# openclimatefix/predict_pv_yield

Hardware: AMD Instinct MI355X
Metric: PV-site samples/sec (train step), conv3d 12->6 frames (higher is better)
Workload: dtype bf16; 1 GPU; conv3d train step (fwd + NMAE + bwd + Adam): sat [B,11,18,64,64] N(0,1), 4x Conv3d(3x3x3, 32ch) + fc 128/128/64, 128.6 M params; per_gpu_batch=32, global_batch=32, t_frames=18, parallelism=single

## Files before the change

include/pv_yield_hip.h:

```cpp
#ifndef PV_YIELD_HIP_H
#define PV_YIELD_HIP_H

#include <stddef.h>
#include <stdint.h>

#ifdef __cplusplus
extern "C" {
#endif

#define PV_ABI_VERSION 1

enum {
  PV_OK = 0,
  PV_EINVAL = -1,
  PV_ESIZE = -2,
  PV_ELAUNCH = -3
};

enum { PV_BORDER_CONSTANT = 0, PV_BORDER_REPLICATE = 1 };

enum {
  PV_U8_ROUND_DIV4 = 0,
  PV_U8_TRUNC_SCALE = 1
};
// ... 481 lines not shown
int pv_layernorm_bwd_workspace_bytes(int64_t rows, int32_t d, size_t* bytes);
int pv_layernorm_bwd_f32(const float* x, const float* w, const float* dy, const float* mean, const float* rstd, float* dx,
                         float* dw, float* db, int64_t rows, int32_t d, void* ws, size_t ws_bytes, int32_t accumulate,
                         const float* dx_add, void* stream);
int pv_layernorm_bwd_params_from_proj_workspace_bytes(int64_t rows, int32_t d, size_t* bytes);
int pv_layernorm_bwd_params_from_proj_bf16(const uint16_t* dkv16, const float* w_kv, const float* x, const float* mean,
                                           const float* rstd, float* dw, float* db, int64_t rows, int32_t d, int32_t kdim,
                                           void* ws, size_t ws_bytes, int32_t accumulate, void* stream);
int pv_context_fwd_bf16(const float* x, const float* x2, int32_t d1, int64_t period, const float* ln_w, const float* ln_b,
                        const float* w_kv, uint16_t* kv16, float* mean, float* rstd, int64_t rows, int32_t d, int32_t kdim,
                        float eps, void* stream);
int pv_context_bwd_workspace_bytes(int64_t rows, int32_t d, size_t* bytes);
int pv_context_bwd_bf16(const uint16_t* dkv16, const float* w_kv, const float* x, const float* x2, int32_t d1, int64_t period,
                        const float* mean, const float* rstd, const float* ln_w, const float* ln_b, float* dw_kv, float* dln_w,
                        float* dln_b, int64_t rows, int32_t d, int32_t kdim, void* ws, size_t ws_bytes, int32_t accumulate_kv,
                        int32_t accumulate_ln, void* stream);
int pv_softmax_fwd_f32(const float* x, float* y, int64_t rows, int32_t len, float scale, void* stream);
int pv_softmax_bwd_f32(const float* p, const float* dp, float* dx, int64_t rows, int32_t len, float scale, void* stream);
int pv_geglu_fwd_f32(const float* x, float* y, int64_t rows, int32_t h, void* stream);
int pv_geglu_bwd_f32(const float* x, const float* dy, float* dx, int64_t rows, int32_t h, void* stream);
int pv_mean_axis1_fwd_f32(const float* x, float* y, int32_t b, int32_t n, int32_t d, void* stream);
int pv_mean_axis1_bwd_f32(const float* dy, float* dx, int32_t b, int32_t n, int32_t d, void* stream);

int pv_gru_seq_fwd_f32(const float* gi, const float* h0, const float* w_hh, const float* b_hh, float* out, float* saved,
                       int32_t batch, int32_t t_len, int32_t hidden, void* stream);
int pv_gru_seq_bwd_f32(const float* dout, const float* dh_last, const float* h0, const float* out, const float* saved,
                       const float* w_hh, float* dgi, float* dh0, float* dw_hh, float* db_hh, int32_t batch, int32_t t_len,
                       int32_t hidden, void* ws, size_t ws_bytes, void* stream);

int pv_forecast_losses_f32(const float* y_hat, const float* y, int64_t y_row_stride,
                           int64_t y_col_stride, int32_t m, int32_t n, float grad_scale,
                           float* out4, float* grad, float* per_horizon, void* stream);

int pv_adam_step_f32(float* param, const float* grad, float* exp_avg, float* exp_avg_sq,
                     uint16_t* bf16_shadow, size_t n, double lr, double beta1, double beta2,
                     double eps, int32_t step, float grad_scale, void* stream);

int pv_ssim_mean_u8(const uint8_t* im1, int64_t stride1, const uint8_t* im2, int64_t stride2, int64_t n_pairs, int32_t h,
                    int32_t w, double data_range, double* out, void* stream);
int pv_ssim_mean_f32(const float* im1, int64_t stride1, const float* im2, int64_t stride2, int64_t n_pairs, int32_t h,
                     int32_t w, double data_range, double* out, void* stream);

int pv_stage_timing_begin(void);
int pv_stage_timing_end(const char** names, float* ms, int32_t* counts, int32_t capacity, int32_t* n_out);

int pv_calibrate_copy_f32(const float* src, float* dst, size_t n, void* stream);
int pv_calibrate_mfma_bf16(float* sink, int32_t workgroups, int32_t iters, void* stream);

int pv_clock_watch(unsigned long long* samples, int32_t n_samples, int32_t sleep_units, void* stream);

#ifdef __cplusplus
}
#endif
#endif
```

predict_pv_yield_amd/_lib.py:

```python
import ctypes
import os
import subprocess

_PKG = os.path.dirname(os.path.abspath(__file__))
LIB_PATH = os.environ.get("PV_YIELD_LIB") or os.path.join(_PKG, "lib", "libpvyield_hip.so")
CSRC_DIR = os.path.join(_PKG, "csrc")

PV_BORDER_CONSTANT = 0
PV_BORDER_REPLICATE = 1
PV_U8_ROUND_DIV4 = 0
PV_U8_TRUNC_SCALE = 1
PV_OPTFLOW_FARNEBACK_GAUSSIAN = 256

c_i32, c_i64, c_f32, c_f64 = ctypes.c_int32, ctypes.c_int64, ctypes.c_float, ctypes.c_double
c_vp, c_sz, c_int, c_u8 = ctypes.c_void_p, ctypes.c_size_t, ctypes.c_int, ctypes.c_uint8


class FarnebackParams(ctypes.Structure):
    _fields_ = [("pyr_scale", c_f64), ("levels", c_i32), ("winsize", c_i32), ("iterations", c_i32),
                ("poly_n", c_i32), ("poly_sigma", c_f64), ("flags", c_i32)]


class Conv3dDims(ctypes.Structure):
    _fields_ = [("batch", c_i32), ("c_in", c_i32), ("c_out", c_i32), ("t_in", c_i32), ("h_in", c_i32),
                ("w_in", c_i32), ("pad_t", c_i32), ("pad_h", c_i32), ("pad_w", c_i32)]

    def out_shape(self):
        return (self.t_in + 2 * self.pad_t - 2, self.h_in + 2 * self.pad_h - 2, self.w_in + 2 * self.pad_w - 2)


class AdamTensor(ctypes.Structure):
    _fields_ = [("param", c_vp), ("grad", c_vp), ("exp_avg", c_vp), ("exp_avg_sq", c_vp), ("bf16_shadow", c_vp),
                ("n", ctypes.c_uint64)]


class PackJob(ctypes.Structure):
    _fields_ = [("w", c_vp), ("wp", c_vp), ("c_out", c_i32), ("c_in", c_i32), ("transpose_flip", c_i32)]


class GemmDesc(ctypes.Structure):
# ... 199 lines not shown
    "pv_attention_fwd_f32": [c_vp, c_vp, c_vp, c_vp, c_vp, ctypes.POINTER(AttentionDesc), c_vp],
    "pv_attention_bwd_f32": [c_vp, c_vp, c_vp, c_vp, c_vp, c_vp, c_vp, c_vp, c_vp, c_vp, ctypes.POINTER(AttentionDesc), c_vp],
    "pv_attention_fwd_bf16": [c_vp, c_vp, c_vp, c_vp, c_vp, ctypes.POINTER(AttentionDesc), c_vp, c_vp],
    "pv_attention_fwd_bf16kv": [c_vp, c_vp, c_vp, c_vp, c_vp, ctypes.POINTER(AttentionDesc), c_vp, c_vp],
    "pv_attention_fwd_workspace_floats": [ctypes.POINTER(AttentionDesc)],
    "pv_attention_bwd_bf16": [c_vp, c_vp, c_vp, c_vp, c_vp, c_vp, c_vp, c_vp, c_vp, c_vp, ctypes.POINTER(AttentionDesc), c_i32, c_vp],
    "pv_attention_bwd_bf16kv": [c_vp, c_vp, c_vp, c_vp, c_vp, c_vp, c_vp, c_vp, c_vp, c_vp, ctypes.POINTER(AttentionDesc), c_i32, c_vp],
    "pv_attention_bwd_bf16kv16": [c_vp, c_vp, c_vp, c_vp, c_vp, c_vp, c_vp, c_vp, c_vp, c_vp, ctypes.POINTER(AttentionDesc), c_vp],
    "pv_attention_bwd_workspace_floats": [ctypes.POINTER(AttentionDesc)],
    "pv_layernorm_fwd_f32": [c_vp, c_vp, c_vp, c_vp, c_vp, c_vp, c_i64, c_i32, c_f32, c_vp],
    "pv_layernorm_bwd_workspace_bytes": [c_i64, c_i32, ctypes.POINTER(c_sz)],
    "pv_layernorm_bwd_f32": [c_vp, c_vp, c_vp, c_vp, c_vp, c_vp, c_vp, c_vp, c_i64, c_i32, c_vp, c_sz, c_i32, c_vp, c_vp],
    "pv_context_fwd_bf16": [c_vp, c_vp, c_i32, c_i64, c_vp, c_vp, c_vp, c_vp, c_vp, c_vp, c_i64, c_i32, c_i32, ctypes.c_float, c_vp],
    "pv_context_bwd_workspace_bytes": [c_i64, c_i32, ctypes.POINTER(c_sz)],
    "pv_context_bwd_bf16": [c_vp, c_vp, c_vp, c_vp, c_i32, c_i64, c_vp, c_vp, c_vp, c_vp, c_vp, c_vp, c_vp, c_i64, c_i32, c_i32,
                            c_vp, c_sz, c_i32, c_i32, c_vp],
    "pv_layernorm_bwd_params_from_proj_workspace_bytes": [c_i64, c_i32, ctypes.POINTER(c_sz)],
    "pv_layernorm_bwd_params_from_proj_bf16": [c_vp, c_vp, c_vp, c_vp, c_vp, c_vp, c_vp, c_i64, c_i32, c_i32, c_vp, c_sz, c_i32, c_vp],
    "pv_softmax_fwd_f32": [c_vp, c_vp, c_i64, c_i32, c_f32, c_vp],
    "pv_softmax_bwd_f32": [c_vp, c_vp, c_vp, c_i64, c_i32, c_f32, c_vp],
    "pv_geglu_fwd_f32": [c_vp, c_vp, c_i64, c_i32, c_vp],
    "pv_geglu_bwd_f32": [c_vp, c_vp, c_vp, c_i64, c_i32, c_vp],
    "pv_mean_axis1_fwd_f32": [c_vp, c_vp, c_i32, c_i32, c_i32, c_vp],
    "pv_mean_axis1_bwd_f32": [c_vp, c_vp, c_i32, c_i32, c_i32, c_vp],
    "pv_gru_seq_fwd_f32": [c_vp, c_vp, c_vp, c_vp, c_vp, c_vp, c_i32, c_i32, c_i32, c_vp],
    "pv_gru_seq_bwd_f32": [c_vp, c_vp, c_vp, c_vp, c_vp, c_vp, c_vp, c_vp, c_vp, c_vp, c_i32, c_i32, c_i32, c_vp, c_sz, c_vp],
    "pv_embedding_fwd_f32": [c_vp, c_vp, c_vp, c_i32, c_i32, c_i32, c_vp],
    "pv_embedding_bwd_f32": [c_vp, c_vp, c_vp, c_i32, c_i32, c_i32, c_vp],
    "pv_cast_f32_to_bf16": [c_vp, c_vp, c_sz, c_vp],
    "pv_scale_bias_relu_f32": [c_vp, c_vp, c_vp, c_i32, c_i32, c_f32, c_i32, c_vp],
    "pv_relu_gate_f32": [c_vp, c_vp, c_vp, c_sz, c_vp],
    "pv_relu_gate_max_f32": [c_vp, c_vp, c_vp, c_sz, c_vp, c_vp],
    "pv_forecast_losses_f32": [c_vp, c_vp, c_i64, c_i64, c_i32, c_i32, c_f32, c_vp, c_vp, c_vp, c_vp],
    "pv_adam_step_f32": [c_vp, c_vp, c_vp, c_vp, c_vp, c_sz, c_f64, c_f64, c_f64, c_f64, c_i32, c_f32, c_vp],
}
_RESTYPES = {"pv_last_error": ctypes.c_char_p, "pv_conv3d_packed_weight_elems": c_sz, "pv_conv3d_split2_weight_elems": c_sz,
             "pv_linear_fwd_f32_skinny_workspace_bytes": c_sz,
             "pv_attention_bwd_workspace_floats": c_sz, "pv_colsum_workspace_floats": c_sz,
             "pv_attention_fwd_workspace_floats": c_sz}


def build_library(verbose: bool = False) -> str:
    args = ["make", "-C", CSRC_DIR, "-j8"]
    if not verbose:
        args.append("-s")
    subprocess.check_call(args)
    return LIB_PATH


_lib = None


def get_lib():
    global _lib
    if _lib is None:
        if not os.path.exists(LIB_PATH):
            raise RuntimeError(
                f"{LIB_PATH} not found: the HIP extension is not built. Run `python -c 'import __graft_entry__ as g; "
                f"g.build()'` (or `make -C {CSRC_DIR}`). predict_pv_yield_amd has no CPU fallback.")
        import torch
        lib = ctypes.CDLL(LIB_PATH)
        for name, argtypes in SIGNATURES.items():
            fn = getattr(lib, name)
            fn.argtypes = argtypes
            fn.restype = _RESTYPES.get(name, c_int)
        if lib.pv_abi_version() != 1:
# ... 37 lines not shown
```

predict_pv_yield_amd/csrc/dense_f32.hip:

```cpp
#include "adam.h"

namespace pv {

__global__ __launch_bounds__(256) void swap01_segments_kernel(const u32x4* __restrict__ src, u32x4* __restrict__ dst, long long n0,
                                                               long long n1, long long seg16) {
  const size_t total = (size_t)n0 * n1 * seg16, stride = (size_t)gridDim.x * blockDim.x;
  for (size_t i = (size_t)blockIdx.x * blockDim.x + threadIdx.x; i < total; i += stride) {
    const size_t seg = i / seg16, c = i - seg * seg16;
    const size_t i1 = seg / n0, i0 = seg - i1 * n0;
    dst[i] = src[(i0 * n1 + i1) * seg16 + c];
  }
}

constexpr int M_TILE = 8;
constexpr long long SMALL_K = 4096, SMALL_MN = 1 << 16;

__global__ __launch_bounds__(256) void linear_fwd_partial_f32(const float* __restrict__ x,
                                                               const float* __restrict__ w,
                                                               float* __restrict__ partial, int m, int n,
                                                               long long k, long long k_chunk) {
  const int col = blockIdx.x;
  const int ks = blockIdx.y;
  const int m0 = blockIdx.z * M_TILE;
  const long long k0 = (long long)ks * k_chunk;
// ... 235 lines not shown
}

__device__ __forceinline__ void linear_bwd_db_body(const float* __restrict__ dy, const float* __restrict__ ymask,
                                                   float* __restrict__ db, int m, int n, int bx) {
  int col = bx * blockDim.x + threadIdx.x;
  if (col >= n) return;
  float s = 0.f;
  for (int r = 0; r < m; ++r) {
    size_t off = (size_t)r * n + col;
    float v = dy[off];
    if (ymask && !(ymask[off] > 0.f)) v = 0.f;
    s += v;
  }
  db[col] = s;
}

__global__ __launch_bounds__(256) void linear_bwd_small_f32(const float* __restrict__ x, const float* __restrict__ w,
                                                             const float* __restrict__ dy, const float* __restrict__ ymask,
                                                             float* __restrict__ dx, float* __restrict__ dw,
                                                             float* __restrict__ db, int m, int n, long long k, int kb,
                                                             int n_dx, int n_dw) {
  extern __shared__ float g[];
  int blk = blockIdx.x;
  if (blk < n_dx) {
    linear_bwd_dx_body(g, w, dy, ymask, dx, m, n, k, blk % kb, blk / kb);
  } else if (blk < n_dx + n_dw) {
    blk -= n_dx;
    linear_bwd_dw_body(g, x, dy, ymask, dw, m, n, k, blk % kb, blk / kb);
  } else {
    linear_bwd_db_body(dy, ymask, db, m, n, blk - n_dx - n_dw);
  }
}

__global__ __launch_bounds__(256) void linear_fwd_small_f32(const float* __restrict__ x, const float* __restrict__ w,
                                                             const float* __restrict__ bias, float* __restrict__ y, int m,
                                                             int n, int k, int relu) {
  const int i = blockIdx.x * blockDim.x + threadIdx.x;
  if (i >= m * n) return;
  const int r = i / n, col = i - r * n;
  const float* xr = x + (size_t)r * k;
  const float* wr = w + (size_t)col * k;
  float s0 = 0.f, s1 = 0.f, s2 = 0.f, s3 = 0.f;
  int kk = 0;
  if ((((uintptr_t)xr | (uintptr_t)wr) & 15) == 0) {
    for (; kk + 64 <= k; kk += 64) {
      f32x4 xv[16], wv[16];
#pragma unroll
      for (int j = 0; j < 16; ++j) xv[j] = *reinterpret_cast<const f32x4*>(xr + kk + 4 * j), wv[j] = *reinterpret_cast<const f32x4*>(wr + kk + 4 * j);
#pragma unroll
      for (int j = 0; j < 16; ++j) {
        s0 = fmaf(xv[j][0], wv[j][0], s0);
        s1 = fmaf(xv[j][1], wv[j][1], s1);
        s2 = fmaf(xv[j][2], wv[j][2], s2);
        s3 = fmaf(xv[j][3], wv[j][3], s3);
      }
    }
    for (; kk + 32 <= k; kk += 32) {
      f32x4 xv[8], wv[8];
#pragma unroll
      for (int j = 0; j < 8; ++j) xv[j] = *reinterpret_cast<const f32x4*>(xr + kk + 4 * j), wv[j] = *reinterpret_cast<const f32x4*>(wr + kk + 4 * j);
#pragma unroll
      for (int j = 0; j < 8; ++j) {
        s0 = fmaf(xv[j][0], wv[j][0], s0);
        s1 = fmaf(xv[j][1], wv[j][1], s1);
        s2 = fmaf(xv[j][2], wv[j][2], s2);
        s3 = fmaf(xv[j][3], wv[j][3], s3);
      }
    }
  }
  for (; kk + 4 <= k; kk += 4) {
    s0 = fmaf(xr[kk], wr[kk], s0);
    s1 = fmaf(xr[kk + 1], wr[kk + 1], s1);
    s2 = fmaf(xr[kk + 2], wr[kk + 2], s2);
    s3 = fmaf(xr[kk + 3], wr[kk + 3], s3);
  }
  for (; kk < k; ++kk) s0 = fmaf(xr[kk], wr[kk], s0);
  float s = (s0 + s1) + (s2 + s3);
  if (bias) s += bias[col];
  if (relu) s = s > 0.f ? s : 0.f;
  y[i] = s;
}

struct LossWeights { float w[64]; };

__global__ __launch_bounds__(256) void forecast_losses_f32(const float* __restrict__ y_hat, const float* __restrict__ y,
                                                            long long y_row_stride, long long y_col_stride, int m,
                                                            int n, float grad_scale, LossWeights lw,
                                                            float* __restrict__ out4, float* __restrict__ grad,
                                                            float* __restrict__ per_horizon) {
  float s_se = 0.f, s_ae = 0.f, s_wse = 0.f, s_wae = 0.f;
  const int total = m * n;
  const float inv = 1.0f / (float)total;
  for (int i = threadIdx.x; i < total; i += blockDim.x) {
    int r = i / n, c = i - r * n;
    float d = y_hat[i] - y[(long long)r * y_row_stride + (long long)c * y_col_stride];
    float a = fabsf(d);
    s_se += d * d;
    s_ae += a;
    s_wse += lw.w[c] * (d * d);
    s_wae += lw.w[c] * a;
    if (grad) grad[i] = (d > 0.f ? 1.f : (d < 0.f ? -1.f : 0.f)) * inv * grad_scale;
  }
  __shared__ float red[4][4];
  float v[4] = {s_se, s_ae, s_wse, s_wae};
#pragma unroll
  for (int q = 0; q < 4; ++q) {
    float t = v[q];
#pragma unroll
    for (int off = 32; off > 0; off >>= 1) t += __shfl_down(t, off, 64);
    if ((threadIdx.x & 63) == 0) red[threadIdx.x >> 6][q] = t;
  }
  __syncthreads();
  if (threadIdx.x < 4) {
    int q = threadIdx.x;
    out4[q] = (((red[0][q] + red[1][q]) + red[2][q]) + red[3][q]) * inv;
  }
  if (per_horizon && (int)threadIdx.x < n) {
    const int c = threadIdx.x;
    float se = 0.f, ae = 0.f;
    for (int r = 0; r < m; ++r) {
      float d = y_hat[r * n + c] - y[(long long)r * y_row_stride + (long long)c * y_col_stride];
      se += d * d;
      ae += fabsf(d);
    }
    per_horizon[c] = se / (float)m;
    per_horizon[n + c] = ae / (float)m;
  }
}

template <typename GT>
__global__ __launch_bounds__(256) void adam_step_f32(float* __restrict__ p, const GT* __restrict__ g,
                                                      float* __restrict__ m, float* __restrict__ v,
                                                      uint16_t* __restrict__ shadow, size_t n, AdamScalars ad,
                                                      float grad_scale) {
  size_t stride = (size_t)gridDim.x * blockDim.x * 4;
  for (size_t i = ((size_t)blockIdx.x * blockDim.x + threadIdx.x) * 4; i < n; i += stride) {
    if (i + 4 <= n) {
      f32x4 pv4 = *reinterpret_cast<const f32x4*>(p + i);
      f32x4 gv4;
      if constexpr (sizeof(GT) == 4) {
        gv4 = *reinterpret_cast<const f32x4*>(g + i);
      } else {
        const u32x2 raw = *reinterpret_cast<const u32x2*>(g + i);
        gv4[0] = __builtin_bit_cast(float, raw[0] << 16); gv4[1] = __builtin_bit_cast(float, raw[0] & 0xffff0000u);
        gv4[2] = __builtin_bit_cast(float, raw[1] << 16); gv4[3] = __builtin_bit_cast(float, raw[1] & 0xffff0000u);
      }
      f32x4 mv4 = *reinterpret_cast<const f32x4*>(m + i);
      f32x4 vv4 = *reinterpret_cast<const f32x4*>(v + i);
      uint16_t sh[4];
#pragma unroll
      for (int j = 0; j < 4; ++j) {
        float mm = mv4[j], vv = vv4[j], pp = pv4[j];
        adam_update(pp, mm, vv, gv4[j] * grad_scale, ad);
        mv4[j] = mm; vv4[j] = vv; pv4[j] = pp;
        sh[j] = f32_to_bf16_bits(pp);
      }
      *reinterpret_cast<f32x4*>(p + i) = pv4;
      *reinterpret_cast<f32x4*>(m + i) = mv4;
      *reinterpret_cast<f32x4*>(v + i) = vv4;
      if (shadow) {
// ... 98 lines not shown
    float mm = mv[j], v2 = vv[j], pp = pv[j];
    adam_update(pp, mm, v2, gv[j] * grad_scale, ad);
    mv[j] = mm, vv[j] = v2, pv[j] = pp;
    sh[j] = f32_to_bf16_bits(pp);
  }
  if (cnt == 4) {
    *reinterpret_cast<f32x4*>(T.param + i0) = *reinterpret_cast<const f32x4*>(pv);
    *reinterpret_cast<f32x4*>(T.exp_avg + i0) = *reinterpret_cast<const f32x4*>(mv);
    *reinterpret_cast<f32x4*>(T.exp_avg_sq + i0) = *reinterpret_cast<const f32x4*>(vv);
    if (T.bf16_shadow) {
      const u32x2 o = {(uint32_t)sh[0] | ((uint32_t)sh[1] << 16), (uint32_t)sh[2] | ((uint32_t)sh[3] << 16)};
      *reinterpret_cast<u32x2*>(T.bf16_shadow + i0) = o;
    }
  } else {
    for (int j = 0; j < cnt; ++j) {
      T.param[i0 + j] = pv[j], T.exp_avg[i0 + j] = mv[j], T.exp_avg_sq[i0 + j] = vv[j];
      if (T.bf16_shadow) T.bf16_shadow[i0 + j] = sh[j];
    }
  }
}

constexpr long long GEMM_K = 1 << 16;

static long long fwd_k_chunk(long long k, int* k_splits) {
  long long chunk = k >= GEMM_K ? 2048 : 8192;
  long long splits = (k + chunk - 1) / chunk;
  if (splits > 512) { splits = 512; chunk = (k + splits - 1) / splits; }
  if (splits < 1) splits = 1;
  splits = (k + chunk - 1) / chunk;
  *k_splits = (int)splits;
  return chunk;
}

}

using namespace pv;

extern "C" {

int pv_linear_workspace_bytes(int32_t m, int32_t n, int64_t k, size_t* bytes) {
  PV_REQUIRE(bytes && m > 0 && n > 0 && k > 0, PV_EINVAL, "pv_linear_workspace_bytes: bad arguments");
  int ks;
  fwd_k_chunk(k, &ks);
  *bytes = (size_t)ks * m * n * sizeof(float);
  return PV_OK;
}

int pv_linear_fwd_f32(const float* x, const float* w, const float* bias, float* y, int32_t m, int32_t n, int64_t k,
                      int relu, void* workspace, size_t workspace_bytes, void* stream) {
  PV_REQUIRE(x && w && y && workspace, PV_EINVAL, "pv_linear_fwd_f32: null pointer");
  PV_REQUIRE(m > 0 && n > 0 && k > 0, PV_EINVAL, "pv_linear_fwd_f32: bad sizes");
  int ks;
  long long chunk = fwd_k_chunk(k, &ks);
  PV_REQUIRE(workspace_bytes >= (size_t)ks * m * n * sizeof(float), PV_ESIZE, "pv_linear_fwd_f32: workspace too small");
  PV_REQUIRE(n <= 65535 && ks <= 65535, PV_ESIZE, "pv_linear_fwd_f32: n too large");
  hipStream_t st = as_stream(stream);
  if (k <= SMALL_K && (long long)m * n <= SMALL_MN) {
    hipLaunchKernelGGL(linear_fwd_small_f32, dim3((unsigned)((m * n + 255) / 256)), dim3(256), 0, st, x, w, bias, y, m, n, (int)k,
                       relu ? 1 : 0);
    return check_launch("pv_linear_fwd_f32");
  }
  if (k >= GEMM_K && k < (1ll << 31)) {
    pv_gemm_desc d = {m, n, (int32_t)k, k, 1, 1, k, n, 1, 1, 0, 0, 0, 0, 0, 0, ks, (int64_t)m * n};
    const int rc = pv_gemm_f32(x, w, nullptr, (float*)workspace, &d, 0, stream);
    if (rc != PV_OK) return rc;
  } else if (k % 4 == 0 && chunk % 4 == 0 && ((uintptr_t)x % 16) == 0 && ((uintptr_t)w % 16) == 0) {
// ... 41 lines not shown
  if (db) {
    hipLaunchKernelGGL(linear_bwd_db_f32, dim3((unsigned)((n + 255) / 256)), dim3(256), 0, st, dy, y_relu_mask, db, m, n);
  }
  return check_launch("pv_linear_bwd_f32");
}

int pv_relu_gate_f32(const float* dy, const float* y, float* out, size_t n, void* stream) {
  PV_REQUIRE(dy && y && out, PV_EINVAL, "pv_relu_gate_f32: null pointer");
  PV_REQUIRE(n % 4 == 0 && ((uintptr_t)dy % 16) == 0 && ((uintptr_t)y % 16) == 0 && ((uintptr_t)out % 16) == 0, PV_EINVAL,
             "pv_relu_gate_f32: 16-byte aligned buffers of a multiple of 4 elements");
  if (n == 0) return PV_OK;
  hipLaunchKernelGGL(relu_gate_f32_kernel, dim3(stream_grid(n / 4, 256)), dim3(256), 0, as_stream(stream), dy, y, out, n / 4,
                     (uint32_t*)nullptr);
  return check_launch("pv_relu_gate_f32");
}

int pv_relu_gate_max_f32(const float* dy, const float* y, float* out, size_t n, float* state, void* stream) {
  PV_REQUIRE(dy && y && out && state, PV_EINVAL, "pv_relu_gate_max_f32: null pointer");
  PV_REQUIRE(n % 4 == 0 && ((uintptr_t)dy % 16) == 0 && ((uintptr_t)y % 16) == 0 && ((uintptr_t)out % 16) == 0 &&
                 ((uintptr_t)state % 4) == 0, PV_EINVAL,
             "pv_relu_gate_max_f32: 16-byte aligned buffers of a multiple of 4 elements");
  hipStream_t st = as_stream(stream);
  PV_REQUIRE(hipMemsetAsync(state, 0, sizeof(uint32_t), st) == hipSuccess, PV_ELAUNCH, "pv_relu_gate_max_f32: memset failed");
  if (n == 0) return PV_OK;
  hipLaunchKernelGGL(relu_gate_f32_kernel, dim3(std::min<unsigned>(stream_grid(n / 4, 256), 4 * kNumCU)), dim3(256), 0, st, dy, y, out,
                     n / 4, reinterpret_cast<uint32_t*>(state));
  return check_launch("pv_relu_gate_max_f32");
}

int pv_forecast_losses_f32(const float* y_hat, const float* y, int64_t y_row_stride, int64_t y_col_stride, int32_t m,
                           int32_t n, float grad_scale, float* out4, float* grad, float* per_horizon, void* stream) {
  PV_REQUIRE(y_hat && y && out4, PV_EINVAL, "pv_forecast_losses_f32: null pointer");
  PV_REQUIRE(m > 0 && n > 0 && n <= 64, PV_ESIZE, "pv_forecast_losses_f32: forecast length %d outside 1..64", n);
  LossWeights lw;
  float tmp[64];
  float sum = 0.f;
  for (int i = 0; i < n; ++i) { tmp[i] = (float)exp(-0.6931471805599453 * i); sum += tmp[i]; }
  for (int i = 0; i < 64; ++i) lw.w[i] = i < n ? tmp[i] / sum * (float)n : 0.f;
  hipLaunchKernelGGL(forecast_losses_f32, dim3(1), dim3(256), 0, as_stream(stream), y_hat, y, (long long)y_row_stride,
                     (long long)y_col_stride, m, n, grad_scale, lw, out4, grad, per_horizon);
  return check_launch("pv_forecast_losses_f32");
}

int pv_swap01_segments(const void* src, void* dst, int64_t n0, int64_t n1, int64_t seg_bytes, void* stream) {
  PV_REQUIRE(src && dst && src != dst, PV_EINVAL, "pv_swap01_segments: null pointer / in place");
  PV_REQUIRE(n0 > 0 && n1 > 0 && seg_bytes > 0 && seg_bytes % 16 == 0, PV_ESIZE,
             "pv_swap01_segments: n0, n1 > 0 and segments of a multiple of 16 bytes, got %lld x %lld x %lld", (long long)n0,
             (long long)n1, (long long)seg_bytes);
  PV_REQUIRE((((uintptr_t)src | (uintptr_t)dst) & 15) == 0, PV_EINVAL, "pv_swap01_segments: buffers must be 16-byte aligned");
  const size_t total = (size_t)n0 * n1 * (seg_bytes / 16);
  hipLaunchKernelGGL(swap01_segments_kernel, dim3(stream_grid(total, 256)), dim3(256), 0, as_stream(stream),
                     static_cast<const u32x4*>(src), static_cast<u32x4*>(dst), (long long)n0, (long long)n1, (long long)(seg_bytes / 16));
  return check_launch("pv_swap01_segments");
}

int pv_cast_f32_to_bf16(const float* src, uint16_t* dst, size_t n, void* stream) {
  PV_REQUIRE(src && dst, PV_EINVAL, "pv_cast_f32_to_bf16: null pointer");
  PV_REQUIRE(((uintptr_t)src % 16 == 0) && ((uintptr_t)dst % 8 == 0), PV_EINVAL, "pv_cast_f32_to_bf16: unaligned");
  if (n == 0) return PV_OK;
  hipLaunchKernelGGL(cast_f32_to_bf16_kernel, dim3(stream_grid((n + 3) / 4, 256)), dim3(256), 0, as_stream(stream), src,
                     dst, n);
  return check_launch("pv_cast_f32_to_bf16");
}

int pv_scale_bias_relu_f32(const float* x, const float* bias, float* y, int32_t m, int32_t n, float alpha, int32_t relu,
                           void* stream) {
  PV_REQUIRE(x && y, PV_EINVAL, "pv_scale_bias_relu_f32: null pointer");
  PV_REQUIRE(m >= 0 && n > 0, PV_ESIZE, "pv_scale_bias_relu_f32: bad sizes");
  const size_t total = (size_t)m * (size_t)n;
  if (total == 0) return PV_OK;
  hipLaunchKernelGGL(scale_bias_relu_kernel, dim3(stream_grid(total, 256)), dim3(256), 0, as_stream(stream), x, bias, y, total, n,
                     alpha, relu);
  return check_launch("pv_scale_bias_relu_f32");
}
// ... 106 lines not shown
```

predict_pv_yield_amd/functional.py:

```python
import ctypes

import torch

from . import hip_ops as K
from . import _large_param as L
from ._backward_pass import PassTable
from ._lib import check, current_stream_ptr, get_lib, ptr


LINEAR_F32_GEMM_K = 1 << 16
F32_PENDING_MAX_ROWS = 1024


def exact_f32() -> bool:
    import os
    return bool(os.environ.get("PV_EXACT_F32"))


class LinearF32(torch.autograd.Function):
    @staticmethod
    def forward(ctx, x, weight, bias, relu):
        x = x.contiguous()
        if (not exact_f32() and x.dtype == torch.float32 and weight.is_contiguous()
                and K.linear_f32_skinny_covers(x.shape[0], weight.shape[0], x.shape[1])):
# ... 547 lines not shown
    t = _UNIT_GRADIENTS.get(key)
    if t is None:
        t = torch.ones((), dtype=loss.dtype, device=loss.device)
        _UNIT_GRADIENTS[key] = t
    return t


class ForecastLosses(torch.autograd.Function):

    @staticmethod
    def forward(ctx, y_hat, y):
        y_hat = y_hat.contiguous()
        out4, grad = K.forecast_losses(y_hat, y, need_grad=True)
        ctx.save_for_backward(grad)
        ctx.set_materialize_grads(False)
        mse, nmae, mse_exp, mae_exp = out4.unbind(0)
        ctx.mark_non_differentiable(mse, mse_exp, mae_exp)
        return mse, nmae, mse_exp, mae_exp

    @staticmethod
    def backward(ctx, g_mse, g_nmae, g_mse_exp, g_mae_exp):
        (grad,) = ctx.saved_tensors
        if g_nmae is None:
            return None, None
        if any(g_nmae is u for u in _UNIT_GRADIENTS.values()):
            return grad, None
        return grad * g_nmae, None


def forecast_losses(y_hat, y):
    return ForecastLosses.apply(y_hat, y)


def forecast_losses_with_horizons(y_hat, y):
    out4, _, horizons = K.forecast_losses(y_hat.detach().contiguous(), y, need_grad=False, per_horizon=True)
    return tuple(out4.unbind(0)), horizons[0], horizons[1]
```

predict_pv_yield_amd/hip_ops.py:

```python
import ctypes
from typing import Callable, NamedTuple, Optional, Sequence

import numpy as np
import torch

from . import _lib
from ._lib import (Conv3dDims, Conv3dGeom, FarnebackParams, PV_BORDER_CONSTANT, PV_BORDER_REPLICATE,
                   PV_OPTFLOW_FARNEBACK_GAUSSIAN, check, current_stream_ptr, get_lib, ptr, require_cuda)

c_i32, c_i64, c_f32, c_f64, c_sz = ctypes.c_int32, ctypes.c_int64, ctypes.c_float, ctypes.c_double, ctypes.c_size_t


def u8_from_10bit(x: torch.Tensor, mode: int = 0, return_flag: bool = False):
    require_cuda(x)
    out = torch.empty(x.shape, dtype=torch.uint8, device=x.device)
    flag = torch.zeros(1, dtype=torch.int32, device=x.device)
    lib = get_lib()
    if x.dtype == torch.int16:
        fn = lib.pv_u8_from_10bit_i16
    elif x.dtype == torch.float32:
        fn = lib.pv_u8_from_10bit_f32
    else:
        raise TypeError(f"u8_from_10bit: int16 or float32 expected, got {x.dtype}")
    check(fn(ptr(x), ptr(out), x.numel(), mode, ptr(flag), current_stream_ptr()), "pv_u8_from_10bit")
# ... 586 lines not shown
    y = torch.empty((m, n), dtype=torch.float32, device=x_bf16.device)
    for r0 in range(0, m, cap):
        rows = min(cap, m - r0)
        check(lib.pv_linear_fwd_bf16(ptr(x_bf16[r0:r0 + rows]), ptr(w_bf16), ptr(bias), ptr(y[r0:r0 + rows]), rows, n, k, int(relu),
                                     ptr(ws), ws.numel(), current_stream_ptr()), "pv_linear_fwd_bf16")
    return y


def linear_bwd_bf16(x_bf16, w_bf16, dy, y_mask, need_dx=True, need_dw=True, gate_dx_by_x=False, need_db=True):
    require_cuda(x_bf16, w_bf16, dy, y_mask)
    m, k = x_bf16.shape
    n = w_bf16.shape[0]
    dx = torch.empty((m, k), dtype=torch.bfloat16, device=dy.device) if need_dx else None
    dw = torch.empty((n, k), dtype=torch.float32, device=dy.device) if need_dw else None
    db = torch.empty(n, dtype=torch.float32, device=dy.device) if need_db else None
    check(get_lib().pv_linear_bwd_bf16(ptr(x_bf16), ptr(w_bf16), ptr(dy), ptr(y_mask), ptr(dx), ptr(dw), ptr(db), m, n,
                                       k, int(bool(gate_dx_by_x and need_dx)), current_stream_ptr()), "pv_linear_bwd_bf16")
    return dx, dw, db


def forecast_losses(y_hat: torch.Tensor, y: torch.Tensor, need_grad: bool = True, grad_scale: float = 1.0,
                    per_horizon: bool = False):
    require_cuda(y_hat)
    if not y.is_cuda or y.dtype != torch.float32 or y.dim() != 2 or y.shape != y_hat.shape:
        raise TypeError("forecast_losses: y must be a float32 CUDA [B, forecast_len] view matching y_hat")
    m, n = y_hat.shape
    out4 = torch.empty(4, dtype=torch.float32, device=y_hat.device)
    grad = torch.empty_like(y_hat) if need_grad else None
    horizons = torch.empty((2, n), dtype=torch.float32, device=y_hat.device) if per_horizon else None
    check(get_lib().pv_forecast_losses_f32(ptr(y_hat), ctypes.c_void_p(y.data_ptr()), y.stride(0), y.stride(1), m, n,
                                           grad_scale, ptr(out4), ptr(grad), ptr(horizons), current_stream_ptr()),
          "pv_forecast_losses_f32")
    return (out4, grad, horizons) if per_horizon else (out4, grad)


def adam_step(param, grad, exp_avg, exp_avg_sq, step: int, lr=5e-4, betas=(0.9, 0.999), eps=1e-8,
              bf16_shadow=None, grad_scale=1.0):
    require_cuda(param, grad, exp_avg, exp_avg_sq, bf16_shadow)
    check(get_lib().pv_adam_step_f32(ptr(param), ptr(grad), ptr(exp_avg), ptr(exp_avg_sq), ptr(bf16_shadow),
                                     param.numel(), lr, betas[0], betas[1], eps, step, grad_scale,
                                     current_stream_ptr()), "pv_adam_step_f32")


def adam_step_multi(items, step: int, lr=5e-4, betas=(0.9, 0.999), eps=1e-8, grad_scale=1.0):
    lib = get_lib()
    for i in range(0, len(items), _lib.PV_ADAM_MAX_TENSORS):
        chunk = items[i:i + _lib.PV_ADAM_MAX_TENSORS]
        arr = (_lib.AdamTensor * len(chunk))()
        for j, (p, g, m, v, sh) in enumerate(chunk):
            require_cuda(p, g, m, v, sh)
            arr[j] = _lib.AdamTensor(ptr(p), ptr(g), ptr(m), ptr(v), ptr(sh), p.numel())
        check(lib.pv_adam_step_multi_f32(arr, len(chunk), lr, betas[0], betas[1], eps, step, grad_scale,
                                         current_stream_ptr()), "pv_adam_step_multi_f32")


def adam_scalars_advance(scalars: torch.Tensor, step: torch.Tensor, lr=5e-4, betas=(0.9, 0.999), eps=1e-8) -> None:
    require_cuda(scalars, step)
    if scalars.dtype != torch.float32 or scalars.numel() < 6 or step.dtype != torch.int32:
        raise TypeError("adam_scalars_advance: float32 [6] scalars and an int32 step on the device")
    check(get_lib().pv_adam_scalars_advance(ptr(scalars), ptr(step), lr, betas[0], betas[1], eps, current_stream_ptr()),
          "pv_adam_scalars_advance")


def adam_step_multi_dev(items, scalars: torch.Tensor, grad_scale=1.0):
    lib = get_lib()
    require_cuda(scalars)
# ... 1570 lines not shown
```

predict_pv_yield_amd/models/base_model.py:

```python
import logging
import os

import numpy as np
import torch

from ..data.batch import BatchML
from ..lightning import LightningModule

logger = logging.getLogger(__name__)

default_output_variable = "pv_yield"


RESULTS_COLUMNS = ("t0_datetime_utc", "target_datetime_utc", "gsp_id", "actual_gsp_pv_outturn_mw",
                   "forecast_gsp_pv_outturn_mw")


def _weighted_losses_weights(n: int, device) -> torch.Tensor:
    w = torch.tensor([float(np.exp(-np.log(2.0) * i)) for i in range(n)], dtype=torch.float32, device=device)
    return w / w.sum() * n


class BaseModel(LightningModule):
    batch_size = 32
# ... 11 lines not shown
        if not hasattr(self, "output_variable"):
            self.output_variable = default_output_variable
        if self.output_variable == "pv_yield":
            self.forecast_len = self.forecast_len_5
            self.history_len = self.history_len_5
            self.number_of_samples_per_batch = 128
        else:
            self.forecast_len = self.forecast_len_30
            self.history_len = self.history_len_30
            self.number_of_samples_per_batch = 32
        self.number_of_pv_samples_per_batch = 128

    def _target(self, batch: BatchML) -> torch.Tensor:
        y = batch.gsp.gsp_yield if self.output_variable == "gsp_yield" else batch.pv.pv_yield
        return y[0 : self.batch_size, -self.forecast_len :, 0]

    def _is_parameter_free(self) -> bool:
        return next(self.parameters(), None) is None

    def _losses(self, y_hat: torch.Tensor, y: torch.Tensor, per_horizon: bool = False):
        if y_hat.is_cuda:
            from ..functional import forecast_losses, forecast_losses_with_horizons
            if per_horizon:
                return forecast_losses_with_horizons(y_hat.float(), y.float())
            return forecast_losses(y_hat.float(), y.float())
        if not self._is_parameter_free():
            raise RuntimeError("predict_pv_yield_amd: losses run on the MI355X only (no CPU path); model is on "
                               f"{y_hat.device}")
        d = y_hat.float() - y.float()
        w = _weighted_losses_weights(d.shape[1], d.device)
        four = ((d * d).mean(), d.abs().mean(), (w * d * d).mean(), (w * d.abs()).mean())
        return (four, (d * d).mean(dim=0), d.abs().mean(dim=0)) if per_horizon else four

    def _training_or_validation_step(self, batch, tag: str, return_model_outputs: bool = False):
        if type(batch) == dict:
            batch = BatchML(**batch)
        y_hat = self(batch)
        y = self._target(batch)
        evaluating = tag != "Train"
        if evaluating:
            (mse_loss, nmae_loss, mse_exp, mae_exp), mse_h, mae_h = self._losses(y_hat, y, per_horizon=True)
        else:
            mse_loss, nmae_loss, mse_exp, mae_exp = self._losses(y_hat, y)
        self.log_dict({f"MSE/{tag}": mse_loss, f"NMAE/{tag}": nmae_loss, f"MSE_EXP/{tag}": mse_exp,
                       f"MAE_EXP/{tag}": mae_exp}, on_step=True, on_epoch=True, sync_dist=True)
        if evaluating:
            metrics_mse = {f"MSE_forecast_horizon_{i}/{tag}": mse_h[i] for i in range(self.forecast_len_30)}
            metrics_mae = {f"MSE_forecast_horizon_{i}/{tag}": mae_h[i] for i in range(self.forecast_len_30)}
            merged = {**metrics_mse, **metrics_mae}
            if merged:
                self.log_dict(merged, on_step=True, on_epoch=True, sync_dist=True)
        if return_model_outputs:
            return nmae_loss, y_hat
        return nmae_loss

    def training_step(self, batch, batch_idx):
        return self._training_or_validation_step(batch, tag="Train")

    def validation_step(self, batch, batch_idx):
        if type(batch) == dict:
            batch = BatchML(**batch)
        nmae_loss, model_output = self._training_or_validation_step(batch, tag="Validation", return_model_outputs=True)
        gsp = getattr(batch, "gsp", None)
        n30 = self.forecast_len_30
        if gsp is not None and getattr(gsp, "gsp_capacity", None) is not None and n30 > 0 and model_output.shape[1] >= n30:
            capacity = gsp.gsp_capacity[:, -n30:, 0].cpu().numpy()
            predictions = model_output[:, -n30:].detach().float().cpu().numpy() * capacity
            truths = gsp.gsp_yield[:, -n30:, 0].cpu().numpy() * capacity
            t0 = batch.metadata.t0_datetime_utc if batch.metadata is not None else None
            if isinstance(t0, torch.Tensor):
                t0 = t0.cpu().numpy()
            elif t0 is not None:
                t0 = np.asarray(t0)
            gsp_ids = gsp.gsp_id[:, 0].cpu().numpy()
            rows = []
            for b in range(predictions.shape[0]):
# ... 31 lines not shown
```

predict_pv_yield_amd/models/conv3d/model.py:

```python
import logging

import torch
from torch import nn

from ...data.batch import BatchML
from ..base_model import BaseModel

logging.basicConfig()
_LOG = logging.getLogger("predict_pv_yield_amd")


FC1_CHANNELS_LAST = True


class Model(BaseModel):

    name = "conv3d"

    def __init__(
        self,
        include_pv_yield: bool = True,
        include_nwp: bool = True,
        forecast_minutes: int = 30,
        history_minutes: int = 60,
# ... 72 lines not shown

    def _mark_fc1_layout(self) -> None:
        from . import _fc1_layout
        _fc1_layout.mark(self)

    def _apply(self, fn, *args, **kwargs):
        out = super()._apply(fn, *args, **kwargs)
        self._mark_fc1_layout()
        return out

    def __setstate__(self, state):
        super().__setstate__(state)
        self._mark_fc1_layout()

    def _bf16_supported(self) -> bool:
        from ._tower import bf16_tower_supported
        return bf16_tower_supported(self.number_sat_channels, self.conv3d_channels, self.cnn_output_size)

    def _satellite_input(self, x: BatchML) -> torch.Tensor:
        sat = x.satellite.data
        if self.future_frames == "optical_flow":
            if getattr(sat, "_pv_advected", False):
                return sat
            if sat.dtype == torch.int16:
                from ...optical_flow import advect_future_frames
                if sat.dim() != 5 or sat.shape[1] != self.history_len_5 + 1 or sat.shape[2] != self.number_sat_channels:
                    raise ValueError(f"raw satellite counts must be [B, {self.history_len_5 + 1}, "
                                     f"{self.number_sat_channels}, H, W] int16, got {tuple(sat.shape)}")
                return advect_future_frames(sat, n_future=self.forecast_len_5)
            from ...optical_flow import replace_future_frames_with_flow
            return replace_future_frames_with_flow(sat.float(), n_future=self.forecast_len_5)
        return sat.float()

    def forward(self, x):
        if type(x) == dict:
            x = BatchML(**x)
        sat_data = self._satellite_input(x)
        from ... import functional as Fn
        from ._tower import conv_tower_fc1
        self._mark_fc1_layout()

        batch_size = sat_data.shape[0]
        out = conv_tower_fc1(sat_data, self._conv_layers(), self.fc1, self.number_sat_channels, self.conv3d_channels,
                             (0, 0, 0), self.cnn_output_size, self.precision == "bf16" and self._bf16_supported(),
                             fc1_channels_last=bool(self._fc1_k_channels))
        out = Fn.linear_f32(out, self.fc2.weight, self.fc2.bias, relu=True)

        if self.include_pv_yield:
            pv_yield_history = x[self.output_variable][:, : self.history_len_30 + 1].nan_to_num(nan=0.0).float()
            pv_yield_history = pv_yield_history.reshape(pv_yield_history.shape[0],
                                                        pv_yield_history.shape[1] * pv_yield_history.shape[2])
            out = torch.cat((out, pv_yield_history), dim=1)
        if self.include_nwp:
            nwp_data = x["nwp"].float().flatten(start_dim=1)
            out_nwp = Fn.linear_f32(nwp_data, self.fc_nwp.weight, self.fc_nwp.bias, relu=True)
            out = torch.cat((out, out_nwp), dim=1)

        out = Fn.linear_f32(out, self.fc3.weight, self.fc3.bias, relu=True)
        out = Fn.linear_f32(out, self.fc4.weight, self.fc4.bias, relu=False)
        return out.reshape(batch_size, self.forecast_len)
```

Baseline: 20320 samples/s.

## Fuse fc2-fc4 head forward and loss into one kernel for training

```diff
diff --git a/include/pv_yield_hip.h b/include/pv_yield_hip.h
--- a/include/pv_yield_hip.h
+++ b/include/pv_yield_hip.h
@@ -537,6 +537,10 @@
                            int64_t y_col_stride, int32_t m, int32_t n, float grad_scale,
                            float* out4, float* grad, float* per_horizon, void* stream);
 
+int pv_dense_head_fwd_f32(const float* a1, const float* w2, const float* b2, const float* w3, const float* b3, const float* w4,
+                          const float* b4, float* a2, float* a3, float* y_hat, const float* y, int64_t y_row_stride,
+                          int64_t y_col_stride, int32_t m, int32_t n1, int32_t n2, int32_t n3, int32_t n4, float grad_scale,
+                          float* out4, float* grad, uint32_t* counter, void* stream);
 int pv_adam_step_f32(float* param, const float* grad, float* exp_avg, float* exp_avg_sq,
                      uint16_t* bf16_shadow, size_t n, double lr, double beta1, double beta2,
                      double eps, int32_t step, float grad_scale, void* stream);
diff --git a/predict_pv_yield_amd/_lib.py b/predict_pv_yield_amd/_lib.py
--- a/predict_pv_yield_amd/_lib.py
+++ b/predict_pv_yield_amd/_lib.py
@@ -6,6 +6,7 @@
 LIB_PATH = os.environ.get("PV_YIELD_LIB") or os.path.join(_PKG, "lib", "libpvyield_hip.so")
 CSRC_DIR = os.path.join(_PKG, "csrc")
 
+PV_ESIZE = -2
 PV_BORDER_CONSTANT = 0
 PV_BORDER_REPLICATE = 1
 PV_U8_ROUND_DIV4 = 0
@@ -271,6 +272,7 @@
     "pv_relu_gate_f32": [c_vp, c_vp, c_vp, c_sz, c_vp],
     "pv_relu_gate_max_f32": [c_vp, c_vp, c_vp, c_sz, c_vp, c_vp],
     "pv_forecast_losses_f32": [c_vp, c_vp, c_i64, c_i64, c_i32, c_i32, c_f32, c_vp, c_vp, c_vp, c_vp],
+    "pv_dense_head_fwd_f32": [c_vp] * 11 + [c_i64, c_i64] + [c_i32] * 5 + [c_f32, c_vp, c_vp, c_vp, c_vp],
     "pv_adam_step_f32": [c_vp, c_vp, c_vp, c_vp, c_vp, c_sz, c_f64, c_f64, c_f64, c_f64, c_i32, c_f32, c_vp],
 }
 _RESTYPES = {"pv_last_error": ctypes.c_char_p, "pv_conv3d_packed_weight_elems": c_sz, "pv_conv3d_split2_weight_elems": c_sz,
diff --git a/predict_pv_yield_amd/csrc/dense_f32.hip b/predict_pv_yield_amd/csrc/dense_f32.hip
--- a/predict_pv_yield_amd/csrc/dense_f32.hip
+++ b/predict_pv_yield_amd/csrc/dense_f32.hip
@@ -291,62 +291,63 @@
   }
 }
 
+__device__ __forceinline__ float linear_fwd_small_body(const float* xr, const float* wr, const float* bias, int col, int k, int relu) {
+  float s0 = 0.f, s1 = 0.f, s2 = 0.f, s3 = 0.f;
+  int kk = 0;
+  if ((((uintptr_t)xr | (uintptr_t)wr) & 15) == 0) {
+    for (; kk + 64 <= k; kk += 64) {
+      f32x4 xv[16], wv[16];
+#pragma unroll
+      for (int j = 0; j < 16; ++j) xv[j] = *reinterpret_cast<const f32x4*>(xr + kk + 4 * j), wv[j] = *reinterpret_cast<const f32x4*>(wr + kk + 4 * j);
+#pragma unroll
+      for (int j = 0; j < 16; ++j) {
+        s0 = fmaf(xv[j][0], wv[j][0], s0);
+        s1 = fmaf(xv[j][1], wv[j][1], s1);
+        s2 = fmaf(xv[j][2], wv[j][2], s2);
+        s3 = fmaf(xv[j][3], wv[j][3], s3);
+      }
+    }
+    for (; kk + 32 <= k; kk += 32) {
+      f32x4 xv[8], wv[8];
+#pragma unroll
+      for (int j = 0; j < 8; ++j) xv[j] = *reinterpret_cast<const f32x4*>(xr + kk + 4 * j), wv[j] = *reinterpret_cast<const f32x4*>(wr + kk + 4 * j);
+#pragma unroll
+      for (int j = 0; j < 8; ++j) {
+        s0 = fmaf(xv[j][0], wv[j][0], s0);
+        s1 = fmaf(xv[j][1], wv[j][1], s1);
+        s2 = fmaf(xv[j][2], wv[j][2], s2);
+        s3 = fmaf(xv[j][3], wv[j][3], s3);
+      }
+    }
+  }
+  for (; kk + 4 <= k; kk += 4) {
+    s0 = fmaf(xr[kk], wr[kk], s0);
+    s1 = fmaf(xr[kk + 1], wr[kk + 1], s1);
+    s2 = fmaf(xr[kk + 2], wr[kk + 2], s2);
+    s3 = fmaf(xr[kk + 3], wr[kk + 3], s3);
+  }
+  for (; kk < k; ++kk) s0 = fmaf(xr[kk], wr[kk], s0);
+  float s = (s0 + s1) + (s2 + s3);
+  if (bias) s += bias[col];
+  if (relu) s = s > 0.f ? s : 0.f;
+  return s;
+}
+
 __global__ __launch_bounds__(256) void linear_fwd_small_f32(const float* __restrict__ x, const float* __restrict__ w,
                                                              const float* __restrict__ bias, float* __restrict__ y, int m,
                                                              int n, int k, int relu) {
   const int i = blockIdx.x * blockDim.x + threadIdx.x;
   if (i >= m * n) return;
   const int r = i / n, col = i - r * n;
-  const float* xr = x + (size_t)r * k;
-  const float* wr = w + (size_t)col * k;
-  float s0 = 0.f, s1 = 0.f, s2 = 0.f, s3 = 0.f;
-  int kk = 0;
-  if ((((uintptr_t)xr | (uintptr_t)wr) & 15) == 0) {
-    for (; kk + 64 <= k; kk += 64) {
-      f32x4 xv[16], wv[16];
-#pragma unroll
-      for (int j = 0; j < 16; ++j) xv[j] = *reinterpret_cast<const f32x4*>(xr + kk + 4 * j), wv[j] = *reinterpret_cast<const f32x4*>(wr + kk + 4 * j);
-#pragma unroll
-      for (int j = 0; j < 16; ++j) {
-        s0 = fmaf(xv[j][0], wv[j][0], s0);
-        s1 = fmaf(xv[j][1], wv[j][1], s1);
-        s2 = fmaf(xv[j][2], wv[j][2], s2);
-        s3 = fmaf(xv[j][3], wv[j][3], s3);
-      }
-    }
-    for (; kk + 32 <= k; kk += 32) {
-      f32x4 xv[8], wv[8];
-#pragma unroll
-      for (int j = 0; j < 8; ++j) xv[j] = *reinterpret_cast<const f32x4*>(xr + kk + 4 * j), wv[j] = *reinterpret_cast<const f32x4*>(wr + kk + 4 * j);
-#pragma unroll
-      for (int j = 0; j < 8; ++j) {
-        s0 = fmaf(xv[j][0], wv[j][0], s0);
-        s1 = fmaf(xv[j][1], wv[j][1], s1);
-        s2 = fmaf(xv[j][2], wv[j][2], s2);
-        s3 = fmaf(xv[j][3], wv[j][3], s3);
-      }
-    }
-  }
-  for (; kk + 4 <= k; kk += 4) {
-    s0 = fmaf(xr[kk], wr[kk], s0);
-    s1 = fmaf(xr[kk + 1], wr[kk + 1], s1);
-    s2 = fmaf(xr[kk + 2], wr[kk + 2], s2);
-    s3 = fmaf(xr[kk + 3], wr[kk + 3], s3);
-  }
-  for (; kk < k; ++kk) s0 = fmaf(xr[kk], wr[kk], s0);
-  float s = (s0 + s1) + (s2 + s3);
-  if (bias) s += bias[col];
-  if (relu) s = s > 0.f ? s : 0.f;
-  y[i] = s;
+  y[i] = linear_fwd_small_body(x + (size_t)r * k, w + (size_t)col * k, bias, col, k, relu);
 }
 
 struct LossWeights { float w[64]; };
 
-__global__ __launch_bounds__(256) void forecast_losses_f32(const float* __restrict__ y_hat, const float* __restrict__ y,
-                                                            long long y_row_stride, long long y_col_stride, int m,
-                                                            int n, float grad_scale, LossWeights lw,
-                                                            float* __restrict__ out4, float* __restrict__ grad,
-                                                            float* __restrict__ per_horizon) {
+__device__ __forceinline__ void forecast_losses_body(const float* y_hat, const float* __restrict__ y, long long y_row_stride,
+                                                     long long y_col_stride, int m, int n, float grad_scale, const LossWeights& lw,
+                                                     float* __restrict__ out4, float* __restrict__ grad,
+                                                     float* __restrict__ per_horizon) {
   float s_se = 0.f, s_ae = 0.f, s_wse = 0.f, s_wae = 0.f;
   const int total = m * n;
   const float inv = 1.0f / (float)total;
@@ -385,6 +386,60 @@
     per_horizon[c] = se / (float)m;
     per_horizon[n + c] = ae / (float)m;
   }
+}
+
+__global__ __launch_bounds__(256) void forecast_losses_f32(const float* __restrict__ y_hat, const float* __restrict__ y,
+                                                            long long y_row_stride, long long y_col_stride, int m,
+                                                            int n, float grad_scale, LossWeights lw,
+                                                            float* __restrict__ out4, float* __restrict__ grad,
+                                                            float* __restrict__ per_horizon) {
+  forecast_losses_body(y_hat, y, y_row_stride, y_col_stride, m, n, grad_scale, lw, out4, grad, per_horizon);
+}
+
+constexpr int HEAD_ROWS = 2;
+
+__device__ __forceinline__ void head_fwd_layer(const float* x, const float* __restrict__ w, const float* __restrict__ bias,
+                                               float* y, int rows, int n, int k, int relu) {
+  for (int i = threadIdx.x; i < rows * n; i += blockDim.x) {
+    const int r = i / n, col = i - r * n;
+    y[i] = linear_fwd_small_body(x + (size_t)r * k, w + (size_t)col * k, bias, col, k, relu);
+  }
+}
+
+struct HeadFwdLayers {
+  const float* w[3];
+  const float* b[3];
+  float* y[3];
+  int n[4];
+};
+
+__global__ __launch_bounds__(256) void dense_head_fwd_f32(const float* __restrict__ a1, HeadFwdLayers L, int m,
+                                                           const float* __restrict__ y, long long y_row_stride,
+                                                           long long y_col_stride, float grad_scale, LossWeights lw,
+                                                           float* __restrict__ out4, float* __restrict__ grad,
+                                                           unsigned int* counter) {
+  const int r0 = blockIdx.x * HEAD_ROWS;
+  const int rows = m - r0 < HEAD_ROWS ? m - r0 : HEAD_ROWS;
+  const float* x = a1 + (size_t)r0 * L.n[0];
+#pragma unroll 1
+  for (int l = 0; l < 3; ++l) {
+    float* out = L.y[l] + (size_t)r0 * L.n[l + 1];
+    head_fwd_layer(x, L.w[l], L.b[l], out, rows, L.n[l + 1], L.n[l], l < 2);
+    __syncthreads();
+    x = out;
+  }
+  __shared__ int is_last;
+  __threadfence();
+  __syncthreads();
+  if (threadIdx.x == 0) {
+    const unsigned int arrived = atomicAdd(counter, 1u);
+    is_last = arrived == gridDim.x - 1;
+    if (is_last) atomicExch(counter, 0u);
+  }
+  __syncthreads();
+  if (!is_last) return;
+  __builtin_amdgcn_fence(__ATOMIC_ACQUIRE, "agent");
+  forecast_losses_body(L.y[2], y, y_row_stride, y_col_stride, m, L.n[3], grad_scale, lw, out4, grad, nullptr);
 }
 
 template <typename GT>
@@ -549,6 +604,15 @@
   return chunk;
 }
 
+static LossWeights weighted_losses_weights(int n) {
+  LossWeights lw;
+  float tmp[64];
+  float sum = 0.f;
+  for (int i = 0; i < n; ++i) { tmp[i] = (float)exp(-0.6931471805599453 * i); sum += tmp[i]; }
+  for (int i = 0; i < 64; ++i) lw.w[i] = i < n ? tmp[i] / sum * (float)n : 0.f;
+  return lw;
+}
+
 }
 
 using namespace pv;
@@ -656,14 +720,35 @@
                            int32_t n, float grad_scale, float* out4, float* grad, float* per_horizon, void* stream) {
   PV_REQUIRE(y_hat && y && out4, PV_EINVAL, "pv_forecast_losses_f32: null pointer");
   PV_REQUIRE(m > 0 && n > 0 && n <= 64, PV_ESIZE, "pv_forecast_losses_f32: forecast length %d outside 1..64", n);
-  LossWeights lw;
-  float tmp[64];
-  float sum = 0.f;
-  for (int i = 0; i < n; ++i) { tmp[i] = (float)exp(-0.6931471805599453 * i); sum += tmp[i]; }
-  for (int i = 0; i < 64; ++i) lw.w[i] = i < n ? tmp[i] / sum * (float)n : 0.f;
   hipLaunchKernelGGL(forecast_losses_f32, dim3(1), dim3(256), 0, as_stream(stream), y_hat, y, (long long)y_row_stride,
-                     (long long)y_col_stride, m, n, grad_scale, lw, out4, grad, per_horizon);
+                     (long long)y_col_stride, m, n, grad_scale, weighted_losses_weights(n), out4, grad, per_horizon);
   return check_launch("pv_forecast_losses_f32");
+}
+
+static int dense_head_covers(const char* who, int32_t m, int32_t n1, int32_t n2, int32_t n3, int32_t n4,
+                             std::initializer_list<const void*> buffers) {
+  PV_REQUIRE(m > 0 && n1 > 0 && n2 > 0 && n3 > 0 && n4 > 0, PV_EINVAL, "%s: bad sizes", who);
+  PV_REQUIRE(m <= 32 && n1 <= SMALL_K && n2 <= 2048 && n3 <= 2048 && n4 <= 64, PV_ESIZE,
+             "%s: m = %d, widths %d -> %d -> %d -> %d outside m <= 32, %lld -> 2048 -> 2048 -> 64", who, m, n1, n2, n3, n4, SMALL_K);
+  uintptr_t bits = 0;
+  for (const void* p : buffers) bits |= (uintptr_t)p;
+  PV_REQUIRE((bits & 15) == 0, PV_ESIZE, "%s: buffers must be 16-byte aligned", who);
+  return PV_OK;
+}
+
+int pv_dense_head_fwd_f32(const float* a1, const float* w2, const float* b2, const float* w3, const float* b3, const float* w4,
+                          const float* b4, float* a2, float* a3, float* y_hat, const float* y, int64_t y_row_stride,
+                          int64_t y_col_stride, int32_t m, int32_t n1, int32_t n2, int32_t n3, int32_t n4, float grad_scale,
+                          float* out4, float* grad, uint32_t* counter, void* stream) {
+  PV_REQUIRE(a1 && w2 && b2 && w3 && b3 && w4 && b4 && a2 && a3 && y_hat && y && out4 && grad && counter, PV_EINVAL,
+             "pv_dense_head_fwd_f32: null pointer");
+  const int rc = dense_head_covers("pv_dense_head_fwd_f32", m, n1, n2, n3, n4, {a1, w2, b2, w3, b3, w4, b4, a2, a3, y_hat, out4, grad});
+  if (rc != PV_OK) return rc;
+  const HeadFwdLayers layers = {{w2, w3, w4}, {b2, b3, b4}, {a2, a3, y_hat}, {n1, n2, n3, n4}};
+  hipLaunchKernelGGL(dense_head_fwd_f32, dim3((unsigned)((m + HEAD_ROWS - 1) / HEAD_ROWS)), dim3(256), 0, as_stream(stream), a1, layers,
+                     m, y, (long long)y_row_stride, (long long)y_col_stride, grad_scale, weighted_losses_weights(n4), out4, grad,
+                     counter);
+  return check_launch("pv_dense_head_fwd_f32");
 }
 
 int pv_swap01_segments(const void* src, void* dst, int64_t n0, int64_t n1, int64_t seg_bytes, void* stream) {
diff --git a/predict_pv_yield_amd/functional.py b/predict_pv_yield_amd/functional.py
--- a/predict_pv_yield_amd/functional.py
+++ b/predict_pv_yield_amd/functional.py
@@ -603,6 +603,41 @@
     return ForecastLosses.apply(y_hat, y)
 
 
+class DenseHeadLosses(torch.autograd.Function):
+
+    @staticmethod
+    def forward(ctx, a1, w2, b2, w3, b3, w4, b4, y):
+        a1, w2, b2, w3, b3, w4, b4 = (t.contiguous() for t in (a1, w2, b2, w3, b3, w4, b4))
+        out = K.dense_head_fwd(a1, w2, b2, w3, b3, w4, b4, y)
+        if out is None:
+            a2 = K.linear_fwd_f32(a1, w2, b2, True)
+            a3 = K.linear_fwd_f32(a2, w3, b3, True)
+            out4, grad = K.forecast_losses(K.linear_fwd_f32(a3, w4, b4, False), y, need_grad=True)
+        else:
+            a2, a3, _, out4, grad = out
+        ctx.save_for_backward(a1, w2, w3, w4, a2, a3, grad)
+        ctx.set_materialize_grads(False)
+        mse, nmae, mse_exp, mae_exp = out4.unbind(0)
+        ctx.mark_non_differentiable(mse, mse_exp, mae_exp)
+        return mse, nmae, mse_exp, mae_exp
+
+    @staticmethod
+    def backward(ctx, g_mse, g_nmae, g_mse_exp, g_mae_exp):
+        a1, w2, w3, w4, a2, a3, g4 = ctx.saved_tensors
+        if g_nmae is None:
+            return (None,) * 8
+        if not any(g_nmae is u for u in _UNIT_GRADIENTS.values()):
+            g4 = g4 * g_nmae
+        dx3, dw4, db4 = K.linear_bwd_f32(a3, w4, g4, None)
+        dx2, dw3, db3 = K.linear_bwd_f32(a2, w3, dx3, a3)
+        dx1, dw2, db2 = K.linear_bwd_f32(a1, w2, dx2, a2)
+        return dx1, dw2, db2, dw3, db3, dw4, db4, None
+
+
+def dense_head_losses(a1, fc2, fc3, fc4, y):
+    return DenseHeadLosses.apply(a1, fc2.weight, fc2.bias, fc3.weight, fc3.bias, fc4.weight, fc4.bias, y)
+
+
 def forecast_losses_with_horizons(y_hat, y):
     out4, _, horizons = K.forecast_losses(y_hat.detach().contiguous(), y, need_grad=False, per_horizon=True)
     return tuple(out4.unbind(0)), horizons[0], horizons[1]
diff --git a/predict_pv_yield_amd/hip_ops.py b/predict_pv_yield_amd/hip_ops.py
--- a/predict_pv_yield_amd/hip_ops.py
+++ b/predict_pv_yield_amd/hip_ops.py
@@ -642,6 +642,32 @@
                                            grad_scale, ptr(out4), ptr(grad), ptr(horizons), current_stream_ptr()),
           "pv_forecast_losses_f32")
     return (out4, grad, horizons) if per_horizon else (out4, grad)
+
+
+_dense_head_counters = {}
+
+
+def dense_head_fwd(a1, w2, b2, w3, b3, w4, b4, y, grad_scale: float = 1.0):
+    require_cuda(a1, w2, b2, w3, b3, w4, b4)
+    m, n1 = a1.shape
+    n2, n3, n4 = w2.shape[0], w3.shape[0], w4.shape[0]
+    if (w2.shape[1], w3.shape[1], w4.shape[1]) != (n1, n2, n3):
+        raise TypeError("dense_head_fwd: weight shapes do not chain")
+    if not y.is_cuda or y.dtype != torch.float32 or y.dim() != 2 or tuple(y.shape) != (m, n4):
+        raise TypeError("dense_head_fwd: y must be a float32 CUDA [B, forecast_len] view matching fc4's output")
+    counter = _dense_head_counters.get(a1.device)
+    if counter is None:
+        counter = _dense_head_counters[a1.device] = torch.zeros(1, dtype=torch.int32, device=a1.device)
+    a2, a3, y_hat = (torch.empty((m, n), dtype=torch.float32, device=a1.device) for n in (n2, n3, n4))
+    out4 = torch.empty(4, dtype=torch.float32, device=a1.device)
+    grad = torch.empty_like(y_hat)
+    rc = get_lib().pv_dense_head_fwd_f32(ptr(a1), ptr(w2), ptr(b2), ptr(w3), ptr(b3), ptr(w4), ptr(b4), ptr(a2), ptr(a3), ptr(y_hat),
+                                         ctypes.c_void_p(y.data_ptr()), y.stride(0), y.stride(1), m, n1, n2, n3, n4, grad_scale,
+                                         ptr(out4), ptr(grad), ptr(counter), current_stream_ptr())
+    if rc == _lib.PV_ESIZE:
+        return None
+    check(rc, "pv_dense_head_fwd_f32")
+    return a2, a3, y_hat, out4, grad
 
 
 def adam_step(param, grad, exp_avg, exp_avg_sq, step: int, lr=5e-4, betas=(0.9, 0.999), eps=1e-8,
diff --git a/predict_pv_yield_amd/models/base_model.py b/predict_pv_yield_amd/models/base_model.py
--- a/predict_pv_yield_amd/models/base_model.py
+++ b/predict_pv_yield_amd/models/base_model.py
@@ -67,16 +67,23 @@
         four = ((d * d).mean(), d.abs().mean(), (w * d * d).mean(), (w * d.abs()).mean())
         return (four, (d * d).mean(dim=0), d.abs().mean(dim=0)) if per_horizon else four
 
+    def _train_losses(self, batch: BatchML):
+        return None
+
     def _training_or_validation_step(self, batch, tag: str, return_model_outputs: bool = False):
         if type(batch) == dict:
             batch = BatchML(**batch)
-        y_hat = self(batch)
-        y = self._target(batch)
         evaluating = tag != "Train"
-        if evaluating:
-            (mse_loss, nmae_loss, mse_exp, mae_exp), mse_h, mae_h = self._losses(y_hat, y, per_horizon=True)
+        four = None if (evaluating or return_model_outputs) else self._train_losses(batch)
+        if four is not None:
+            mse_loss, nmae_loss, mse_exp, mae_exp = four
         else:
-            mse_loss, nmae_loss, mse_exp, mae_exp = self._losses(y_hat, y)
+            y_hat = self(batch)
+            y = self._target(batch)
+            if evaluating:
+                (mse_loss, nmae_loss, mse_exp, mae_exp), mse_h, mae_h = self._losses(y_hat, y, per_horizon=True)
+            else:
+                mse_loss, nmae_loss, mse_exp, mae_exp = self._losses(y_hat, y)
         self.log_dict({f"MSE/{tag}": mse_loss, f"NMAE/{tag}": nmae_loss, f"MSE_EXP/{tag}": mse_exp,
                        f"MAE_EXP/{tag}": mae_exp}, on_step=True, on_epoch=True, sync_dist=True)
         if evaluating:
diff --git a/predict_pv_yield_amd/models/conv3d/model.py b/predict_pv_yield_amd/models/conv3d/model.py
--- a/predict_pv_yield_amd/models/conv3d/model.py
+++ b/predict_pv_yield_amd/models/conv3d/model.py
@@ -128,18 +128,31 @@
             return replace_future_frames_with_flow(sat.float(), n_future=self.forecast_len_5)
         return sat.float()
 
+    def _tower_fc1(self, x: BatchML) -> torch.Tensor:
+        sat_data = self._satellite_input(x)
+        from ._tower import conv_tower_fc1
+        self._mark_fc1_layout()
+        return conv_tower_fc1(sat_data, self._conv_layers(), self.fc1, self.number_sat_channels, self.conv3d_channels,
+                              (0, 0, 0), self.cnn_output_size, self.precision == "bf16" and self._bf16_supported(),
+                              fc1_channels_last=bool(self._fc1_k_channels))
+
+    def _head_is_plain(self) -> bool:
+        import os
+        return (self.precision == "bf16" and not self.include_pv_yield and not self.include_nwp
+                and type(self).forward is Model.forward and not os.environ.get("PV_DENSE_HEAD_PER_LAYER"))
+
+    def _train_losses(self, batch: BatchML):
+        if not self._head_is_plain():
+            return None
+        from ... import functional as Fn
+        return Fn.dense_head_losses(self._tower_fc1(batch), self.fc2, self.fc3, self.fc4, self._target(batch).float())
+
     def forward(self, x):
         if type(x) == dict:
             x = BatchML(**x)
-        sat_data = self._satellite_input(x)
         from ... import functional as Fn
-        from ._tower import conv_tower_fc1
-        self._mark_fc1_layout()
-
-        batch_size = sat_data.shape[0]
-        out = conv_tower_fc1(sat_data, self._conv_layers(), self.fc1, self.number_sat_channels, self.conv3d_channels,
-                             (0, 0, 0), self.cnn_output_size, self.precision == "bf16" and self._bf16_supported(),
-                             fc1_channels_last=bool(self._fc1_k_channels))
+        out = self._tower_fc1(x)
+        batch_size = out.shape[0]
         out = Fn.linear_f32(out, self.fc2.weight, self.fc2.bias, relu=True)
 
         if self.include_pv_yield:
```

After: 20390 samples/s (median of 4 runs). Within noise of the previous version (+0.3%).
